# Diegotistical/OptionsLab

Hardware: AMD Instinct MI355X
Metric: MC path-steps/sec (1M paths × 252 steps Euro call); price vs BS |err|/σ (higher is better)
Workload: dtype f32 normals / f64 prices

## Files before the change

include/olmc.h:

```cpp
#ifndef OLMC_H
#define OLMC_H

#include <stdint.h>

#ifdef __cplusplus
extern "C" {
#endif

#define OLMC_ABI_VERSION 6

enum {
    OLMC_OK = 0,
    OLMC_ERR_ARG = 1,
    OLMC_ERR_HIP = 2,
    OLMC_ERR_STATE = 3,
    OLMC_ERR_RCCL = 4
};

enum { OLMC_STREAM_GBM = 0, OLMC_STREAM_HESTON = 1, OLMC_STREAM_JUMP = 2, OLMC_STREAM_KOU = 3 };
enum { OLMC_AVG_ARITHMETIC = 0, OLMC_AVG_GEOMETRIC = 1, OLMC_AVG_ARITHMETIC_FAST = 2 };
#define OLMC_MAX_BATCH 16

typedef struct olmc_stats {
    double  sum;
// ... 184 lines not shown
                       const uint32_t* sv, const uint32_t* shift, int32_t bits, int path_major, double* out_host);

int olmc_multi_gpu_european(double S, double K, double T, double r, double sigma, double q, int is_call,
                            int64_t n_paths, int32_t n_steps, uint64_t seed, int antithetic,
                            int n_gpus, olmc_stats* out);
int olmc_multi_gpu_greeks_fd(double S, double K, double T, double r, double sigma, double q, int is_call,
                             int64_t n_paths, int32_t n_steps, uint64_t seed, int second_order,
                             int n_gpus, double* out9, olmc_stats* evals );
int olmc_multi_gpu_european_cv(double S, double K, double T, double r, double sigma, double q, int is_call,
                               int64_t n_paths, int32_t n_steps, uint64_t seed, int antithetic,
                               int n_gpus, olmc_cv_moments* out);
int olmc_multi_gpu_european_qmc(double S, double K, double T, double r, double sigma, double q, int is_call,
                                int64_t n_paths, int32_t dims, const uint32_t* sv, const uint32_t* shift, int32_t bits,
                                int n_gpus, olmc_stats* out);
int olmc_multi_gpu_european_qmc_greeks_fd(double S, double K, double T, double r, double sigma, double q, int is_call,
                                          int64_t n_paths, int32_t dims, const uint32_t* sv, const uint32_t* shift, int32_t bits,
                                          int second_order, int n_gpus, double* out9, olmc_stats* evals );
int olmc_multi_gpu_european_qmc_cv(double S, double K, double T, double r, double sigma, double q, int is_call,
                                   int64_t n_paths, int32_t dims, const uint32_t* sv, const uint32_t* shift, int32_t bits,
                                   int n_gpus, olmc_cv_moments* out);
int olmc_multi_gpu_spans(double* out8);

int olmc_fetch_dev(const double* d_src, int32_t n, void* hip_stream, double* out_host);

int olmc_combine_stats(const olmc_stats* parts, int32_t n_parts, double r, double T, olmc_stats* out);

int olmc_philox_words(uint64_t seed, int64_t path_offset, int64_t n_paths,
                      int32_t block0, int32_t n_blocks, uint32_t stream_tag, uint32_t* out_host);
int olmc_normals(uint64_t seed, int64_t path_offset, int64_t n_paths, int32_t n_steps,
                 float* out_host);

int olmc_profile_enable(int on);
enum { OLMC_TUNE_GRID_CAP = 2, OLMC_TUNE_QMC_BLOCK = 4, OLMC_TUNE_SPLIT_TAIL = 7, OLMC_TUNE_POLL = 8, OLMC_TUNE_SPLIT_SAT = 9,
       OLMC_TUNE_MULTI_LAUNCH = 10, OLMC_TUNE_STAGED_COPY = 11 };
int olmc_tune(int knob, int value);
int olmc_profile_reset(void);
int olmc_kernel_time(int64_t* launches, double* total_ms);

#ifdef __cplusplus
}
#endif
#endif
```

optionslab_amd/_hip.py:

```python
from __future__ import annotations

import ctypes as C
import importlib.util
import os
import sys
import threading
from typing import List, Optional, Sequence, Tuple

import numpy as np

from .exceptions import AccelerationError

LIBRARY_PATH = os.environ.get("OLMC_LIBRARY") or os.path.join(os.path.dirname(os.path.abspath(__file__)), "libolmc.so")
MAX_BATCH = 16
AVG_ARITHMETIC, AVG_GEOMETRIC, AVG_ARITHMETIC_FAST = 0, 1, 2
_U64 = (1 << 64) - 1


class Stats(C.Structure):
    _fields_ = [("sum", C.c_double), ("sumsq", C.c_double), ("n", C.c_int64),
                ("price", C.c_double), ("std_error", C.c_double)]


class Option(C.Structure):
# ... 46 lines not shown
    "olmc_extrema_qmc": (_I, _SIX + [_I, _I, _D, _I, _I64, _I64, _I32, C.POINTER(C.c_uint32), C.POINTER(C.c_uint32), _I32, _I, C.POINTER(Stats)]),
    "olmc_asian_qmc_greeks_fd": (_I, _SIX + [_I, _I, _I, _I64, _I32, C.POINTER(C.c_uint32), C.POINTER(C.c_uint32), _I32, _I, _I, C.POINTER(_D), C.POINTER(Stats)]),
    "olmc_extrema_qmc_greeks_fd": (_I, _SIX + [_I, _I, _D, _I, _I64, _I32, C.POINTER(C.c_uint32), C.POINTER(C.c_uint32), _I32, _I, _I, C.POINTER(_D),
                                              C.POINTER(Stats)]),
    "olmc_asian_greeks_fd": (_I, _SIX + [_I, _I, _I64, _I32, _U64T, _I, _I, C.POINTER(_D), C.POINTER(Stats)]),
    "olmc_extrema_greeks_fd": (_I, _SIX + [_I, _I, _D, _I64, _I32, _U64T, _I, _I, C.POINTER(_D), C.POINTER(Stats)]),
    "olmc_barrier": (_I, _SIX + [_I, _D, _I, _I64, _I64, _I32, _U64T, _I, C.POINTER(Stats)]),
    "olmc_lookback": (_I, _SIX + [_I, _I, _I64, _I64, _I32, _U64T, _I, C.POINTER(Stats)]),
    "olmc_autocallable": (_I, [_D] * 9 + [_I32, _I64, _I64, _I32, _U64T, _I, C.POINTER(Stats)]),
    "olmc_cliquet": (_I, [_D] * 9 + [_I32, _I64, _I64, _I32, _U64T, _I, C.POINTER(Stats)]),
    "olmc_exercise_boundary": (_I, _SIX + [_I, _I64, _I32, _U64T, C.POINTER(_D)]),
    "olmc_heston_paths": (_I, [_D] * 9 + [_I64, _I32, _U64T, _I, C.POINTER(_D), C.POINTER(_D)]),
    "olmc_jump_paths": (_I, [_D] * 5 + [_I, _D, _D, _D, _D, _I64, _I32, _U64T, _I, C.POINTER(_D)]),
    "olmc_american_lsm": (_I, _SIX + [_I, _I64, _I32, _I32, _U64T, C.POINTER(Stats)]),
    "olmc_autocallable_qmc": (_I, [_D] * 9 + [_I32, _I, _I64, _I64, _I32, C.POINTER(C.c_uint32), C.POINTER(C.c_uint32), _I32, _I, C.POINTER(Stats)]),
    "olmc_cliquet_qmc": (_I, [_D] * 9 + [_I32, _I, _I64, _I64, _I32, C.POINTER(C.c_uint32), C.POINTER(C.c_uint32), _I32, _I, C.POINTER(Stats)]),
    "olmc_american_lsm_qmc": (_I, _SIX + [_I, _I, _I64, _I32, C.POINTER(C.c_uint32), C.POINTER(C.c_uint32), _I32, _I32, C.POINTER(Stats)]),
    "olmc_exercise_boundary_qmc": (_I, _SIX + [_I, _I, _I64, _I32, C.POINTER(C.c_uint32), C.POINTER(C.c_uint32), _I32, C.POINTER(_D)]),
    "olmc_gbm_qmc_paths": (_I, [_D] * 5 + [_I, _I64, _I32, C.POINTER(C.c_uint32), C.POINTER(C.c_uint32), _I32, _I, C.POINTER(_D)]),
    "olmc_jump_diffusion": (_I, _SIX + [_I, _I, _D, _D, _D, _D, _I64, _I64, _I32, _U64T, C.POINTER(Stats)]),
    "olmc_heston": (_I, [_D] * 5 + [_I] + [_D] * 5 + [_I64, _I64, _I32, _U64T, _I, C.POINTER(Stats)]),
    "olmc_multi_gpu_european": (_I, _SIX + [_I, _I64, _I32, _U64T, _I, _I, C.POINTER(Stats)]),
    "olmc_multi_gpu_greeks_fd": (_I, _SIX + [_I, _I64, _I32, _U64T, _I, _I, C.POINTER(_D), C.POINTER(Stats)]),
    "olmc_multi_gpu_european_cv": (_I, _SIX + [_I, _I64, _I32, _U64T, _I, _I, C.POINTER(CvMoments)]),
    "olmc_multi_gpu_european_qmc": (_I, _SIX + [_I, _I64, _I32, C.POINTER(C.c_uint32), C.POINTER(C.c_uint32), _I32, _I, C.POINTER(Stats)]),
    "olmc_multi_gpu_european_qmc_greeks_fd": (_I, _SIX + [_I, _I64, _I32, C.POINTER(C.c_uint32), C.POINTER(C.c_uint32), _I32, _I, _I, C.POINTER(_D), C.POINTER(Stats)]),
    "olmc_multi_gpu_european_qmc_cv": (_I, _SIX + [_I, _I64, _I32, C.POINTER(C.c_uint32), C.POINTER(C.c_uint32), _I32, _I, C.POINTER(CvMoments)]),
    "olmc_multi_gpu_spans": (_I, [C.POINTER(_D)]),
    "olmc_combine_stats": (_I, [C.POINTER(Stats), _I32, _D, _D, C.POINTER(Stats)]),
    "olmc_philox_words": (_I, [_U64T, _I64, _I64, _I32, _I32, C.c_uint32, C.POINTER(C.c_uint32)]),
    "olmc_normals": (_I, [_U64T, _I64, _I64, _I32, C.POINTER(C.c_float)]),
    "olmc_profile_enable": (_I, [_I]),
    "olmc_tune": (_I, [_I, _I]),
    "olmc_profile_reset": (_I, []),
    "olmc_kernel_time": (_I, [C.POINTER(_I64), C.POINTER(_D)]),
}

_lock = threading.Lock()
_lib: Optional[C.CDLL] = None
_initialised = False


def _share_hip_runtime_with_torch() -> None:
    if "torch" in sys.modules or os.environ.get("OLMC_SYSTEM_HIP") == "1":
        return
    try:
        spec = importlib.util.find_spec("torch")
    except (ImportError, ValueError):
        return
    if spec is None or not spec.submodule_search_locations:
        return
    cand = os.path.join(list(spec.submodule_search_locations)[0], "lib", "libamdhip64.so")
    if os.path.exists(cand):
        try:
            C.CDLL(cand, mode=C.RTLD_GLOBAL)
        except OSError:
            pass


def load_library() -> C.CDLL:
    global _lib
    with _lock:
        if _lib is None:
            _share_hip_runtime_with_torch()
            if not os.path.exists(LIBRARY_PATH):
                raise AccelerationError(
# ... 500 lines not shown
    _check(lib().olmc_multi_gpu_spans(out))
    return dict(zip(("launch_us", "collective_us", "fetch_us", "drain_us", "total_us", "wake_us_max", "rank_launch_us_max", "rank_launch_us_min"), out))


def combine_stats(parts: Sequence[Tuple[float, float, int]], r: float, T: float) -> Stats:
    k = len(parts)
    arr = (Stats * k)(*[Stats(s, ss, int(n), 0.0, 0.0) for (s, ss, n) in parts])
    out = Stats()
    _check(load_library().olmc_combine_stats(arr, k, r, T, C.byref(out)))
    return out


def philox_words(seed: int, path_offset: int, n_paths: int, block0: int, n_blocks: int, tag: int = 0) -> np.ndarray:
    out = np.empty((int(n_paths), int(n_blocks), 4), dtype=np.uint32)
    _check(lib().olmc_philox_words(seed64(seed), int(path_offset), int(n_paths), int(block0), int(n_blocks), int(tag),
                                   out.ctypes.data_as(C.POINTER(C.c_uint32))))
    return out


def normals(seed: int, path_offset: int, n_paths: int, n_steps: int) -> np.ndarray:
    out = np.empty((int(n_paths), int(n_steps)), dtype=np.float32)
    _check(lib().olmc_normals(seed64(seed), int(path_offset), int(n_paths), int(n_steps),
                              out.ctypes.data_as(C.POINTER(C.c_float))))
    return out


TUNE_GRID_CAP = 2
TUNE_QMC_BLOCK = 4
TUNE_SPLIT_TAIL = 7
TUNE_POLL = 8
TUNE_SPLIT_SAT = 9
TUNE_MULTI_LAUNCH = 10
TUNE_STAGED_COPY = 11


def tune(knob: int, value: int) -> None:
    _check(load_library().olmc_tune(int(knob), int(value)))


def profile_enable(on: bool) -> None:
    _check(lib().olmc_profile_enable(int(on)))


def profile_reset() -> None:
    _check(lib().olmc_profile_reset())


def kernel_time() -> Tuple[int, float]:
    n, ms = C.c_int64(0), C.c_double(0.0)
    _check(lib().olmc_kernel_time(C.byref(n), C.byref(ms)))
    return n.value, ms.value
```

optionslab_amd/csrc/olmc.hip:

```cpp
#include "olmc.h"
#include "olmc_kernels.h"
#include "olmc_job_board.h"

#include <dlfcn.h>
#include <sched.h>
#include <time.h>
#include <hip/hip_ext.h>
#include <rccl/rccl.h>

#include <algorithm>
#include <atomic>
#include <chrono>
#include <climits>
#include <condition_variable>
#include <cmath>
#include <cstdio>
#include <cstdlib>
#include <cstring>
#include <functional>
#include <mutex>
#include <string>
#include <system_error>
#include <thread>
#include <vector>
#include <linux/futex.h>
#include <sys/prctl.h>
#include <sys/syscall.h>
#include <unistd.h>

namespace {

using namespace olmc;

thread_local std::string t_error = "";
thread_local int t_device = -1;

int fail(int code, const std::string& msg) {
    t_error = msg;
    return code;
}

#define HIP_TRY(expr)                                                                          \
    do {                                                                                       \
        hipError_t e_ = (expr);                                                                \
        if (e_ != hipSuccess)                                                                  \
            return fail(OLMC_ERR_HIP, std::string(#expr) + ": " + hipGetErrorString(e_));      \
    } while (0)

constexpr int kMaxDevices = 16;
constexpr int kMaxNV = 2 * OLMC_MAX_BATCH;
constexpr int32_t kMaxGrid = 1 << 18;
constexpr int32_t kMaxGroups = kMaxGrid / kGroupBlocks + 1;
static_assert(kMaxGroups * kMaxNV == kGroupRowsCapacity, "device-side guard must match the group_rows allocation");

struct EventPair {
    hipEvent_t start, stop;
};

struct DeviceCtx {
    int device = -1;
    int cus = 0;
    hipStream_t stream = nullptr;
    struct WsSlot {
        double* block_rows = nullptr;
        size_t cap = 0;
        double* group_rows = nullptr;
        uint32_t* counters = nullptr;
        hipEvent_t done = nullptr;
        bool used = false;
        bool claimed = false;
        hipStream_t owner = nullptr;
        bool shared = false;
    };
    static constexpr int kSlots = 8;
    WsSlot slots[kSlots + 1];
    int next_slot = 0, cur_slot = 0;
    uint64_t* h_flag = nullptr;
    uint64_t* d_flag = nullptr;
    uint64_t seq = 0;
    uint64_t armed = 0;
    double* h_result = nullptr;
    double* d_result = nullptr;
    void* d_bulk = nullptr;
    size_t bulk_bytes = 0;
    void* h_stage[2] = {nullptr, nullptr};
    hipEvent_t stage_landed[2] = {nullptr, nullptr};
    void* d_multi = nullptr;
    void* h_multi = nullptr;
    void* d_h_multi = nullptr;
    int64_t multi_cap = 0;
    size_t multi_bpo = 0;
    size_t multi_off_done = 0, multi_off_opts = 0, multi_off_rows = 0, multi_hoff_out = 0;
    uint32_t* d_sobol = nullptr;
    size_t sobol_words = 0;
    std::vector<uint32_t> sobol_host;
    void* d_bridge = nullptr;
    int32_t bridge_n = 0;
    std::vector<unsigned char> bridge_host;
    bool busy = false;
    std::vector<EventPair> ev_free, ev_pending;
    int64_t prof_launches = 0;
    double prof_ms = 0.0;
};

constexpr int kMaxContexts = 8;

struct DevicePool {
    std::mutex mu;
    std::condition_variable idle;
    std::vector<DeviceCtx*> all;
    int device = -1;
};

std::mutex g_mu;
std::atomic<DevicePool*> g_pool[kMaxDevices] = {};
std::atomic<int> g_default_device{-1};
bool g_profile = false;

int ctx_allocate(DeviceCtx* c) {
    HIP_TRY(hipStreamCreateWithFlags(&c->stream, hipStreamNonBlocking));
    for (auto& sl : c->slots) {
        HIP_TRY(hipMalloc(&sl.group_rows, sizeof(double) * kMaxNV * kMaxGroups));
        HIP_TRY(hipMalloc(&sl.counters, sizeof(uint32_t) * (kMaxGroups + 1) * kCounterStride));
        HIP_TRY(hipMemset(sl.counters, 0, sizeof(uint32_t) * (kMaxGroups + 1) * kCounterStride));
        HIP_TRY(hipEventCreateWithFlags(&sl.done, hipEventDisableTiming));
    }
    HIP_TRY(hipHostMalloc(&c->h_result, sizeof(double) * (kMaxNV + 1 + 15), hipHostMallocMapped));
    HIP_TRY(hipHostGetDevicePointer(reinterpret_cast<void**>(&c->d_result), c->h_result, 0));
    c->h_flag = reinterpret_cast<uint64_t*>(c->h_result + kMaxNV + 8);
    c->d_flag = reinterpret_cast<uint64_t*>(c->d_result + kMaxNV + 8);
    *c->h_flag = 0;
    return OLMC_OK;
}

void ctx_release(DeviceCtx* c) {
    if (c->stream) (void)hipStreamSynchronize(c->stream);
    for (auto& ep : c->ev_pending) { (void)hipEventDestroy(ep.start); (void)hipEventDestroy(ep.stop); }
    for (auto& ep : c->ev_free) { (void)hipEventDestroy(ep.start); (void)hipEventDestroy(ep.stop); }
    if (c->d_bulk) (void)hipFree(c->d_bulk);
    for (int i = 0; i < 2; ++i) {
        if (c->h_stage[i]) (void)hipHostFree(c->h_stage[i]);
        if (c->stage_landed[i]) (void)hipEventDestroy(c->stage_landed[i]);
    }
    if (c->d_multi) (void)hipFree(c->d_multi);
    if (c->h_multi) (void)hipHostFree(c->h_multi);
    if (c->d_sobol) (void)hipFree(c->d_sobol);
    if (c->d_bridge) (void)hipFree(c->d_bridge);
    for (auto& sl : c->slots) {
        if (sl.block_rows) (void)hipFree(sl.block_rows);
        if (sl.group_rows) (void)hipFree(sl.group_rows);
        if (sl.counters) (void)hipFree(sl.counters);
        if (sl.done) (void)hipEventDestroy(sl.done);
    }
    if (c->h_result) (void)hipHostFree(c->h_result);
    if (c->stream) (void)hipStreamDestroy(c->stream);
    delete c;
}

int ctx_create(int device, DeviceCtx** out) {
    int count = 0;
    hipError_t e = hipGetDeviceCount(&count);
    if (e != hipSuccess || count <= 0)
        return fail(OLMC_ERR_HIP, std::string("no HIP device available: ") + hipGetErrorString(e));
    if (device < 0 || device >= count || device >= kMaxDevices)
        return fail(OLMC_ERR_ARG, "device index out of range");
    HIP_TRY(hipSetDevice(device));
    hipDeviceProp_t prop;
    HIP_TRY(hipGetDeviceProperties(&prop, device));
    DeviceCtx* c = new DeviceCtx();
    c->device = device;
    c->cus = prop.multiProcessorCount;
    const int rc = ctx_allocate(c);
    if (rc) {
        ctx_release(c);
        return rc;
    }
    *out = c;
    return OLMC_OK;
}

struct CtxLease {
    DeviceCtx* c = nullptr;
    DevicePool* pool = nullptr;
    CtxLease() = default;
    CtxLease(const CtxLease&) = delete;
    CtxLease& operator=(const CtxLease&) = delete;
    ~CtxLease() { release(); }
// ... 120 lines not shown
        if (err == hipSuccess) err = hipEventRecord(c->stage_landed[slot], c->stream);
        if (err == hipSuccess && i >= 1) {
            const auto t = clock::now();
            err = hipEventSynchronize(c->stage_landed[slot ^ 1]);
            if (i == 1) us_first = us_since(t); else us_events += us_since(t);
            if (err == hipSuccess) landed.store(i, std::memory_order_release);
        }
    }
    {
        const auto t = clock::now();
        if (err == hipSuccess) err = hipEventSynchronize(c->stage_landed[(n_chunks - 1) & 1]);
        us_events += us_since(t);
    }
    if (err == hipSuccess) landed.store(n_chunks, std::memory_order_release);
    else give_up.store(true);
    const auto t_join = clock::now();
    for (std::thread& t : threads) t.join();
    if (trace)
        std::fprintf(stderr, "[olmc copy_to_host] %.1f MB, %lld chunks, %d threads: spawn %.0f us, first chunk landed (kernel + DMA) %.0f us, later event waits %.0f us, "
                             "waits for the copy threads %.0f us, last chunk out + join %.0f us, total %.0f us\n", bytes / 1e6, static_cast<long long>(n_chunks), n_threads,
                     us_spawn, us_first, us_events, us_workers, us_since(t_join), us_since(t_begin));
    if (err != hipSuccess) {
        (void)hipStreamSynchronize(c->stream);
        (void)hipGetLastError();
        return fail(OLMC_ERR_HIP, std::string("copy_to_host: ") + hipGetErrorString(err));
    }
    return OLMC_OK;
}

int g_multi_launch = 0;
int g_grid_cap = 0;
int g_qmc_block = 0;
int g_poll = 0;
int g_split_tail = 0;
int g_split_sat = 0;
#ifdef OLMC_WITH_PROBES
int g_fault_shard = 0;
int g_force_nv = 0;
int g_multi_rehearsal = 0;
#endif

constexpr int32_t kShortPathSteps = 128, kShortPathGrid = 4096;

int32_t grid_for(int64_t n_paths, int32_t n_steps = INT32_MAX) {
    int64_t cap = g_grid_cap > 0 ? std::min<int64_t>(g_grid_cap, kMaxGrid) : kMaxGrid;
    if (g_grid_cap == 0 && n_steps <= kShortPathSteps) cap = kShortPathGrid;
    return static_cast<int32_t>(std::min<int64_t>((n_paths + kBlock - 1) / kBlock, cap));
}

template <typename Kernel>
int resident_workgroups(Kernel kernel) {
    static std::mutex mu;
    static std::vector<std::pair<const void*, int>> cache;
    const void* key = reinterpret_cast<const void*>(kernel);
    std::lock_guard<std::mutex> lock(mu);
    for (const auto& e : cache)
        if (e.first == key) return e.second;
    int nb = 0;
    if (hipOccupancyMaxActiveBlocksPerMultiprocessor(&nb, kernel, kBlock, 0) != hipSuccess || nb < 1) {
        (void)hipGetLastError();
        nb = 1;
    }
    cache.emplace_back(key, nb);
    return nb;
}

// ... 40 lines not shown
                HIP_TRY(hipDeviceSynchronize());
                taken.shared = true;
                taken.used = false;
            }
        }
    }
    DeviceCtx::WsSlot& sl = c->slots[idx];
    c->cur_slot = idx;
    const bool guarded = !own && sl.shared;
    const size_t need = static_cast<size_t>(grid) * nv;
    if (need > sl.cap) {
        if (!guarded) HIP_TRY(hipStreamSynchronize(stream));
        else if (sl.used) HIP_TRY(hipEventSynchronize(sl.done));
        if (sl.block_rows) HIP_TRY(hipFree(sl.block_rows));
        sl.block_rows = nullptr;
        sl.cap = 0;
        const size_t cap = std::max<size_t>(need, size_t(1) << 16);
        HIP_TRY(hipMalloc(&sl.block_rows, sizeof(double) * cap));
        sl.cap = cap;
    }
    if (guarded && sl.used) HIP_TRY(hipStreamWaitEvent(stream, sl.done, 0));
    ws->block_rows = sl.block_rows;
    ws->group_rows = sl.group_rows;
    ws->counters = sl.counters;
    ws->out = d_out;
    ws->tail = tail;
    ws->row_capacity = sl.cap;
#ifdef OLMC_WITH_PROBES
    if (g_force_nv > 0) ws->row_capacity = static_cast<uint64_t>(grid) * g_force_nv;
#endif
    ws->done_flag = nullptr;
    ws->done_value = 0;
    c->armed = 0;
    if (own && d_out == c->d_result && g_poll >= 0) {
        c->armed = ++c->seq;
        ws->done_flag = c->d_flag;
        ws->done_value = c->armed;
    }
    return OLMC_OK;
}

void ws_recover(DeviceCtx* c) {
    c->armed = 0;
    (void)hipDeviceSynchronize();
    (void)hipGetLastError();
    for (auto& sl : c->slots) (void)hipMemset(sl.counters, 0, sizeof(uint32_t) * (kMaxGroups + 1) * kCounterStride);
}

void multi_recover(DeviceCtx* c) {
    c->armed = 0;
    (void)hipDeviceSynchronize();
    (void)hipGetLastError();
    if (c->d_multi) (void)hipMemset(c->d_multi, 0, c->multi_off_opts);
}

int after_launch(DeviceCtx* c, hipStream_t stream) {
    hipError_t e = hipGetLastError();
    if (e != hipSuccess) { ws_recover(c); return fail(OLMC_ERR_HIP, std::string("kernel launch: ") + hipGetErrorString(e)); }
    if (c->cur_slot == DeviceCtx::kSlots || !c->slots[c->cur_slot].shared) return OLMC_OK;
    DeviceCtx::WsSlot& sl = c->slots[c->cur_slot];
    HIP_TRY(hipEventRecord(sl.done, stream));
    sl.used = true;
    return OLMC_OK;
}

int prof_begin(DeviceCtx* c, hipStream_t s, EventPair* ep) {
    if (c->ev_free.empty()) {
        HIP_TRY(hipEventCreate(&ep->start));
        HIP_TRY(hipEventCreate(&ep->stop));
    } else {
        *ep = c->ev_free.back();
        c->ev_free.pop_back();
    }
    HIP_TRY(hipEventRecord(ep->start, s));
    return OLMC_OK;
}
// ... 64 lines not shown
template <typename F>
void with_set_anti(int nsets, bool anti, F&& f) {
    with_bool(nsets == 8, [&](auto eight) { with_bool(anti, [&](auto a) { f(std::integral_constant<int, eight ? 8 : 16>{}, a); }); });
}

int prof_pair(DeviceCtx* c, EventPair* ep, const EventPair** timed) {
    *timed = nullptr;
    if (!g_profile) return OLMC_OK;
    int rc = prof_acquire(c, ep);
    if (rc) return rc;
    c->ev_pending.push_back(*ep);
    *timed = ep;
    return OLMC_OK;
}

template <int NSETS, int MODE>
void launch_european(bool anti, int32_t grid, hipStream_t s, const PathRange& pr, const ContractSet<NSETS>& cs,
                     const ReduceWs& ws, double* terminal, const EventPair* timed = nullptr) {
    const bool strided = static_cast<int64_t>(grid) * kBlock < pr.count;
    with_bool(strided, [&](auto strided_c) {
        with_bool(anti, [&](auto a) {
            launch_timed(european_path_kernel<NSETS, a, MODE, strided_c>, dim3(grid), dim3(kBlock), s, timed, pr, cs, ws, terminal);
        });
    });
}

int sync_or_recover(DeviceCtx* c, hipStream_t s);

template <typename Launch>
int launch_reduce(DeviceCtx* c, hipStream_t s, double* d_out, double tail, int nv, int32_t grid, Launch&& launch, bool profiled = true) {
    ReduceWs ws;
    int rc = make_ws(c, s, grid, nv, d_out, tail, &ws);
    if (rc) return rc;
    EventPair ep{};
    const EventPair* timed = nullptr;
    if (profiled) {
        rc = prof_pair(c, &ep, &timed);
        if (rc) return rc;
    }
    launch(grid, s, timed, ws);
    rc = after_launch(c, s);
    if (rc || d_out != c->d_result) return rc;
    return sync_or_recover(c, s);
}

void finish_one(const double* h, int64_t n, double r_disc, double T, bool bad, olmc_stats* out) {
    if (bad) nan_stats(n, out);
    else finish_stats(h[0], h[1], n, r_disc, T, out);
}

void finish_set(const double* h, const int* pos, int64_t n, const olmc_option* opts, int64_t k, bool extra_bad, bool lean, olmc_stats* st) {
    for (int64_t i = 0; i < k; ++i) {
        const int64_t slot = pos ? pos[i] : i;
        const olmc_option& o = opts[i];
        if (extra_bad || poisoned(o.S, o.K, o.T, o.r, o.sigma, o.q)) nan_stats(n, &st[i]);
        else if (lean) finish_stats(h[slot], std::nan(""), n, o.r, o.T, &st[i]);
        else finish_stats(h[2 * slot], h[2 * slot + 1], n, o.r, o.T, &st[i]);
    }
}

struct GbmStep {
    double dt, drift, vol;
};
GbmStep gbm_step(double T, int32_t n_steps, double r, double q, double sigma) {
    const double dt = T / n_steps;
    return {dt, (r - q - 0.5 * sigma * sigma) * dt, sigma * std::sqrt(dt)};
// ... 15 lines not shown
            ContractSet<width> cs;
            group_contracts<width>(opts, k, n_steps, &cs, pos);
            if (!lean) launch_european<width, kReduce>(anti, g, st, pr, cs, ws, nullptr, timed);
            else with_bool(anti, [&](auto a) { launch_timed(european_path_kernel<width, a, kSumOnly, false>, dim3(g), dim3(kBlock), st, timed, pr, cs, ws, nullptr); });
        };
        if (nsets == 1) {
            ContractSet<1> cs;
            cs.c[0] = make_contract(opts[0], n_steps);
            cs.base_mask = 1u; cs.upper_continues_slot0 = 0;
            if (pos) pos[0] = 0;
            launch_european<1, kReduce>(anti, g, st, pr, cs, ws, nullptr, timed);
        } else if (nsets == 8) {
            fused(std::integral_constant<int, 8>{});
        } else {
            fused(std::integral_constant<int, 16>{});
        }
    }, profiled);
}

constexpr int64_t kSpinUs = 200, kYieldUs = 2000, kSleepUs = 20;

struct TimerSlack {
    long old = -1;
    void tighten() {
        if (old >= 0) return;
        old = prctl(PR_GET_TIMERSLACK, 0, 0, 0, 0);
        if (old >= 0 && prctl(PR_SET_TIMERSLACK, 1000UL, 0, 0, 0) != 0) old = -1;
    }
    ~TimerSlack() {
        if (old >= 0) (void)prctl(PR_SET_TIMERSLACK, static_cast<unsigned long>(old), 0, 0, 0);
    }
};

int wait_armed(DeviceCtx* c, hipStream_t s) {
    if (c->armed != 0) {
        const uint64_t want = c->armed;
        c->armed = 0;
        using clock = std::chrono::steady_clock;
        const auto t0 = clock::now();
        bool queried = false;
        int phase = 0;
        TimerSlack slack;
        for (uint32_t spins = 0;; ++spins) {
            if (__atomic_load_n(c->h_flag, __ATOMIC_ACQUIRE) == want) {
                if (queried) (void)hipGetLastError();
                return OLMC_OK;
            }
            if (phase == 0) {
                __builtin_ia32_pause();
                if ((spins & 0x3F) == 0x3F && clock::now() - t0 >= std::chrono::microseconds(kSpinUs)) phase = 1;
                continue;
            }
            if (phase == 1) {
                sched_yield();
                if ((spins & 0xF) == 0xF && clock::now() - t0 >= std::chrono::microseconds(kYieldUs)) phase = 2;
                continue;
            }
            if ((spins & 0x3F) == 0) {
                const hipError_t q = hipStreamQuery(s);
                queried = true;
                if (q == hipSuccess) break;
                if (q != hipErrorNotReady) {
                    ws_recover(c);
                    return fail(OLMC_ERR_HIP, std::string("hipStreamQuery: ") + hipGetErrorString(q));
                }
            }
            slack.tighten();
            const timespec nap{0, kSleepUs * 1000};
            nanosleep(&nap, nullptr);
        }
        (void)hipGetLastError();
    }
    hipError_t e = hipStreamSynchronize(s);
    if (e != hipSuccess) { ws_recover(c); return fail(OLMC_ERR_HIP, std::string("hipStreamSynchronize: ") + hipGetErrorString(e)); }
    return OLMC_OK;
}

int sync_or_recover(DeviceCtx* c, hipStream_t s) {
    if (s != c->stream) c->armed = 0;
    return wait_armed(c, s);
}

int run_batch(const olmc_option* opts, int32_t k, int64_t path_offset, int64_t n_local, int32_t n_steps,
              uint64_t seed, int antithetic, olmc_stats* out, bool prices_only = false) {
    if (!opts || !out) return fail(OLMC_ERR_ARG, "null pointer");
    if (k < 1 || k > OLMC_MAX_BATCH) return fail(OLMC_ERR_ARG, "batch size must be in [1, OLMC_MAX_BATCH]");
    int rc = check_paths(path_offset, n_local, n_steps);
    if (rc) return rc;
    CtxLease lease;
    rc = ctx_lease(&lease);
    if (rc) return rc;
    DeviceCtx* const c = lease.c;
    int pos[OLMC_MAX_BATCH];
    bool lean = prices_only;
    rc = run_batch_device(c, c->stream, opts, k, path_offset, n_local, n_steps, seed, antithetic, c->d_result, -1.0, pos, true, &lean);
    if (rc) return rc;
    finish_set(c->h_result, pos, n_local * (antithetic ? 2 : 1), opts, k, false, lean, out);
    return OLMC_OK;
}

}

namespace { void multi_gpu_release(); }

extern "C" int olmc_abi_version(void) { return OLMC_ABI_VERSION; }

extern "C" const char* olmc_last_error(void) { return t_error.c_str(); }

extern "C" int olmc_init(int device) {
    std::lock_guard<std::mutex> lock(g_mu);
    static const bool env_read = [] {
        const char* p = std::getenv("OLMC_POLL");
        if (p && p[0] == '0') g_poll = -1;
        const char* t = std::getenv("OLMC_SPLIT_TAIL");
        if (t && t[0] == '0') g_split_tail = -1;
        const char* m = std::getenv("OLMC_MULTI_LAUNCH");
        if (m && m[0] == 's') g_multi_launch = -1;
        const char* sc = std::getenv("OLMC_STAGED_COPY");
        if (sc && sc[0] == '0') g_staged_copy = -1;
        return true;
    }();
    (void)env_read;
    if (device < 0 || device >= kMaxDevices) return fail(OLMC_ERR_ARG, "device index out of range");
    if (!g_pool[device].load(std::memory_order_acquire)) {
        DeviceCtx* c = nullptr;
        int rc = ctx_create(device, &c);
        if (rc) return rc;
        DevicePool* pool = new DevicePool();
        pool->device = device;
        pool->all.push_back(c);
        g_pool[device].store(pool, std::memory_order_release);
    } else {
        HIP_TRY(hipSetDevice(device));
    }
    t_device = device;
    if (g_default_device.load() < 0) g_default_device.store(device, std::memory_order_release);
    return OLMC_OK;
}

extern "C" int olmc_shutdown(void) {
    std::lock_guard<std::mutex> lock(g_mu);
    multi_gpu_release();
    for (int d = 0; d < kMaxDevices; ++d) {
        DevicePool* pool = g_pool[d].load();
        if (!pool) continue;
        const bool usable = hipSetDevice(d) == hipSuccess;
// ... 1843 lines not shown
    rc = bulk_reserve(c, bytes);
    if (rc) return rc;
    const int64_t total = n_paths * n_blocks;
    const int grid = static_cast<int>(std::min<int64_t>((total + 255) / 256, 4096));
    hipLaunchKernelGGL(philox_words_kernel, dim3(grid), dim3(256), 0, c->stream, static_cast<uint64_t>(path_offset), n_paths,
                       block0, n_blocks, stream_tag, static_cast<uint32_t>(seed), static_cast<uint32_t>(seed >> 32),
                       static_cast<uint32_t*>(c->d_bulk));
    HIP_TRY(hipGetLastError());
    HIP_TRY(hipMemcpyAsync(out_host, c->d_bulk, bytes, hipMemcpyDeviceToHost, c->stream));
    HIP_TRY(hipStreamSynchronize(c->stream));
    return OLMC_OK;
}

extern "C" int olmc_normals(uint64_t seed, int64_t path_offset, int64_t n_paths, int32_t n_steps, float* out_host) {
    if (!out_host || n_paths < 1 || n_steps < 1 || path_offset < 0) return fail(OLMC_ERR_ARG, "bad arguments");
    CtxLease lease;
    int rc = ctx_lease(&lease);
    if (rc) return rc;
    DeviceCtx* const c = lease.c;
    const size_t bytes = sizeof(float) * static_cast<size_t>(n_paths) * n_steps;
    rc = bulk_reserve(c, bytes);
    if (rc) return rc;
    const int64_t total = n_paths * ((n_steps + 3) / 4);
    const int grid = static_cast<int>(std::min<int64_t>((total + 255) / 256, 4096));
    hipLaunchKernelGGL(normals_kernel, dim3(grid), dim3(256), 0, c->stream, static_cast<uint64_t>(path_offset), n_paths,
                       n_steps, static_cast<uint32_t>(seed), static_cast<uint32_t>(seed >> 32),
                       static_cast<float*>(c->d_bulk));
    HIP_TRY(hipGetLastError());
    HIP_TRY(hipMemcpyAsync(out_host, c->d_bulk, bytes, hipMemcpyDeviceToHost, c->stream));
    HIP_TRY(hipStreamSynchronize(c->stream));
    return OLMC_OK;
}

extern "C" int olmc_tune(int knob, int value) {
    if (knob == OLMC_TUNE_GRID_CAP && value >= 0) { g_grid_cap = value; return OLMC_OK; }
    if (knob == OLMC_TUNE_QMC_BLOCK && value >= -1 && value <= 2) { g_qmc_block = value; return OLMC_OK; }
    if (knob == OLMC_TUNE_POLL && value >= -1 && value <= 0) { g_poll = value; return OLMC_OK; }
    if (knob == OLMC_TUNE_SPLIT_TAIL && value >= -1 && value <= 0) { g_split_tail = value; return OLMC_OK; }
    if (knob == OLMC_TUNE_SPLIT_SAT && value >= 0 && value <= 16) { g_split_sat = value; return OLMC_OK; }
    if (knob == OLMC_TUNE_MULTI_LAUNCH && value >= -1 && value <= 0) { g_multi_launch = value; return OLMC_OK; }
    if (knob == OLMC_TUNE_STAGED_COPY && value >= -1 && value <= 0) { g_staged_copy = value; return OLMC_OK; }
    return fail(OLMC_ERR_ARG, "unknown tuning knob or value");
}

namespace {
template <typename Fn>
int with_all_contexts(Fn fn) {
    int dev = t_device >= 0 ? t_device : g_default_device.load(std::memory_order_acquire);
    if (dev < 0) {
        int rc = olmc_init(0);
        if (rc) return rc;
        dev = t_device;
    }
    DevicePool* pool = g_pool[dev].load(std::memory_order_acquire);
    if (!pool) return fail(OLMC_ERR_STATE, "device not initialised (call olmc_init)");
    HIP_TRY(hipSetDevice(dev));
    std::vector<DeviceCtx*> mine;
    {
        std::unique_lock<std::mutex> lock(pool->mu);
        pool->idle.wait(lock, [&] { return std::none_of(pool->all.begin(), pool->all.end(), [](const DeviceCtx* c) { return c->busy; }); });
        mine = pool->all;
        for (DeviceCtx* c : mine) c->busy = true;
    }
    int rc = OLMC_OK;
    for (DeviceCtx* c : mine) {
        const int r = fn(c);
        if (r && !rc) rc = r;
    }
    {
        std::lock_guard<std::mutex> lock(pool->mu);
// ... 50 lines not shown
```

optionslab_amd/csrc/olmc_host_math.h:

```cpp
#ifndef OLMC_HOST_MATH_H
#define OLMC_HOST_MATH_H

#include "olmc.h"

#include <algorithm>
#include <cmath>
#include <cstdint>
#include <cstring>

namespace olmc {

struct Contract {
    double a;
    double vol;
    double strike;
    double sign;
    double scale;
    double neg_sign_strike;
    double sign_scale;
};

template <int NSETS>
struct ContractSet {
    Contract c[NSETS];
// ... 306 lines not shown
            if (n_groups == real_slots) return "more distinct path recursions than the fused Asian Greeks kernel carries";
            as->drift[g] = drift;
            as->vol[g] = vol;
            ++n_groups;
        }
        as->group[i] = g;
    }
    for (int g = n_groups; g < kAsianGroups; ++g) { as->drift[g] = as->drift[0]; as->vol[g] = as->vol[0]; }
    for (int g = 0; g < kAsianGroups; ++g) {
        as->drift[g] = as->drift[g] * unit;
        as->vol[g] = as->vol[g] * kZScale * unit;
    }
    as->strike = K;
    as->sign = is_call ? 1.0 : -1.0;
    as->inv_steps = 1.0 / n_steps;
    return nullptr;
}

inline void shard_range(int64_t n_paths, int rank, int n_ranks, int64_t* lo, int64_t* count) {
    const int64_t a = n_paths * rank / n_ranks, b = n_paths * (rank + 1) / n_ranks;
    *lo = a;
    *count = b - a;
}

constexpr int64_t kQmcShardAlign = 512, kQmcShardMinPoints = 4096;
inline void qmc_shard_range(int64_t n_points, int rank, int n_ranks, int64_t* lo, int64_t* count) {
    if (n_points / n_ranks < kQmcShardMinPoints) return shard_range(n_points, rank, n_ranks, lo, count);
    const int64_t a = n_points * rank / n_ranks / kQmcShardAlign * kQmcShardAlign;
    const int64_t b = rank + 1 == n_ranks ? n_points : n_points * (rank + 1) / n_ranks / kQmcShardAlign * kQmcShardAlign;
    *lo = a;
    *count = b - a;
}

}

#endif
```

optionslab_amd/csrc/olmc_kernels.h:

```cpp
#pragma once
#include <type_traits>
#include <hip/hip_runtime.h>
#include <stdint.h>

#include "olmc_host_math.h"

namespace olmc {

constexpr int kBlock = 256;
constexpr int kWave = 64;
constexpr int kWavesPerBlock = kBlock / kWave;

constexpr uint32_t kPhiloxM0 = 0xD2511F53u;
constexpr uint32_t kPhiloxM1 = 0xCD9E8D57u;
constexpr uint32_t kPhiloxW0 = 0x9E3779B9u;
constexpr uint32_t kPhiloxW1 = 0xBB67AE85u;

struct Words4 {
    uint32_t x0, x1, x2, x3;
};

__device__ __forceinline__ uint32_t xor3(uint32_t a, uint32_t b, uint32_t c) {
    return __builtin_amdgcn_bitop3_b32(a, b, c, 0x96);
}
// ... 119 lines not shown
            float s = 0.0f;
            for (; b < full; ++b) s = raw_block_sum_of_words(s, philox4x32_10_pinned(g_lo, g_hi, static_cast<uint32_t>(b), tag, rk));
            q += static_cast<double>(s);
        }
        const int32_t rem = n_steps & 3;
        if (rem) {
            const Words4 wd = philox4x32_10_pinned(g_lo, g_hi, static_cast<uint32_t>(full), tag, rk);
            float s = 0.0f;
            if (rem > 1) s = pair_sum_raw(0.0f, wd.x0, wd.x1);
            if (rem & 1) {
                float z_cos, z_sin;
                box_muller_raw(rem == 1 ? wd.x0 : wd.x2, rem == 1 ? wd.x1 : wd.x3, z_cos, z_sin);
                s = __builtin_fmaf(z_cos, kInvSqrt2F, s);
            }
            q += static_cast<double>(s);
        }
        acc += q;
    }
    return acc;
}

__device__ __forceinline__ double path_normal_sum(uint32_t g_lo, uint32_t g_hi, int32_t n_steps, uint32_t k0, uint32_t k1,
                                                  uint32_t tag = 0u) {
    return path_normal_quarters(g_lo, g_hi, n_steps, 0, 4, k0, k1, tag) * kPairZScale;
}

__device__ __forceinline__ double wave_sum(double v) {
#pragma unroll
    for (int off = kWave / 2; off > 0; off >>= 1) v += __shfl_down(v, off, kWave);
    return v;
}

constexpr int kGroupBlocks = 256;
constexpr int kGroupRowsCapacity = ((1 << 18) / kGroupBlocks + 1) * 32;
constexpr int kCounterStride = 64;

struct ReduceWs {
    double* block_rows;
    double* group_rows;
    uint32_t* counters;
    double* out;
    double tail;
    uint64_t row_capacity;
    uint64_t* done_flag;
    uint64_t done_value;
};

__device__ __forceinline__ void signal_done(const ReduceWs& ws) {
    if (ws.done_flag == nullptr) return;
    __builtin_amdgcn_fence(__ATOMIC_RELEASE, "");
    if (threadIdx.x == 0) __hip_atomic_store(ws.done_flag, ws.done_value, __ATOMIC_RELAXED, __HIP_MEMORY_SCOPE_SYSTEM);
}

#ifndef OLMC_AGENT_ACQUIRE
#define OLMC_AGENT_ACQUIRE 1
#endif
#if !OLMC_AGENT_ACQUIRE && defined(__HIP_DEVICE_COMPILE__) && !defined(__gfx942__) && !defined(__gfx950__)
#error "OLMC_AGENT_ACQUIRE=0 relies on gfx942 / gfx950 cache behaviour (sc1 rows are L2-served): build this target with the acquire"
#endif
__device__ __forceinline__ void acquire_rows() {
#if OLMC_AGENT_ACQUIRE
    __builtin_amdgcn_fence(__ATOMIC_ACQUIRE, "agent");
#else
    __builtin_amdgcn_fence(__ATOMIC_ACQUIRE, "wavefront");
#endif
}

__device__ __forceinline__ void store_sc1(double* p, double v) {
    __hip_atomic_store(p, v, __ATOMIC_RELAXED, __HIP_MEMORY_SCOPE_AGENT);
}
__device__ __forceinline__ double load_sc1(const double* p) {
    return __hip_atomic_load(p, __ATOMIC_RELAXED, __HIP_MEMORY_SCOPE_AGENT);
}

template <int NV>
__device__ __forceinline__ double wave_rows_sum(const double* src, int32_t rows) {
    constexpr int NVP = NV <= 2 ? 2 : NV <= 8 ? 8 : NV <= 16 ? 16 : 32;
    constexpr int SUBS = kWave / NVP;
    const int lane = threadIdx.x & (kWave - 1);
    const int c = lane % NVP, sub = lane / NVP;
    double v = 0.0;
    if (c < NV) {
        constexpr int kBatch = 8;
        for (int32_t row = sub; row < rows; row += SUBS * kBatch) {
// ... 1 lines not shown
#pragma unroll
            for (int j = 0; j < kBatch; ++j) {
                const int32_t rj = row + j * SUBS;
                t[j] = rj < rows ? load_sc1(src + static_cast<size_t>(rj) * NV + c) : 0.0;
            }
#pragma unroll
            for (int j = 0; j < kBatch; ++j) v += t[j];
        }
    }
#pragma unroll
    for (int off = kWave / 2; off >= NVP; off >>= 1) v += __shfl_down(v, off, kWave);
    return v;
}

struct NoEpilogue {
    __device__ __forceinline__ void operator()(double) const {}
};

template <int NV, typename Epilogue = NoEpilogue>
__device__ __forceinline__ void grid_reduce(double v, const ReduceWs& ws, Epilogue done = Epilogue()) {
    const int lane = threadIdx.x;
    const int32_t n_blocks = static_cast<int32_t>(gridDim.x);
    const int32_t n_groups = (n_blocks + kGroupBlocks - 1) / kGroupBlocks;
    const int32_t group = static_cast<int32_t>(blockIdx.x) / kGroupBlocks;
    const int32_t group_size = min(kGroupBlocks, n_blocks - group * kGroupBlocks);

    if (static_cast<uint64_t>(n_blocks) * NV > ws.row_capacity || n_groups * NV > kGroupRowsCapacity) {
        if (blockIdx.x == 0) {
            if (lane < NV) ws.out[lane] = __builtin_nan("");
            signal_done(ws);
        }
        return;
    }
    if (lane < NV) store_sc1(ws.block_rows + static_cast<size_t>(blockIdx.x) * NV + lane, v);
    asm volatile("s_waitcnt vmcnt(0)" ::: "memory");
    uint32_t ticket = 0;
    if (lane == 0) ticket = __hip_atomic_fetch_add(ws.counters + static_cast<size_t>(group) * kCounterStride, 1u, __ATOMIC_RELAXED, __HIP_MEMORY_SCOPE_AGENT);
    ticket = __builtin_amdgcn_readfirstlane(ticket);
    if (ticket != static_cast<uint32_t>(group_size - 1)) return;

    acquire_rows();
    const double g = wave_rows_sum<NV>(ws.block_rows + static_cast<size_t>(group) * kGroupBlocks * NV, group_size);
    if (n_groups == 1) {
        if (lane < NV) ws.out[lane] = g;
        if (lane == 0) {
            if (ws.tail >= 0.0) ws.out[NV] = ws.tail;
            __hip_atomic_store(ws.counters, 0u, __ATOMIC_RELAXED, __HIP_MEMORY_SCOPE_AGENT);
        }
        done(g);
        signal_done(ws);
        return;
    }
    if (lane < NV) store_sc1(ws.group_rows + static_cast<size_t>(group) * NV + lane, g);
    asm volatile("s_waitcnt vmcnt(0)" ::: "memory");
    if (lane == 0) {
        __hip_atomic_store(ws.counters + static_cast<size_t>(group) * kCounterStride, 0u, __ATOMIC_RELAXED, __HIP_MEMORY_SCOPE_AGENT);
        ticket = __hip_atomic_fetch_add(ws.counters + static_cast<size_t>(n_groups) * kCounterStride, 1u, __ATOMIC_RELAXED, __HIP_MEMORY_SCOPE_AGENT);
    }
    ticket = __builtin_amdgcn_readfirstlane(ticket);
    if (ticket != static_cast<uint32_t>(n_groups - 1)) return;

    acquire_rows();
    const double total = wave_rows_sum<NV>(ws.group_rows, n_groups);
    if (lane < NV) ws.out[lane] = total;
    if (lane == 0) {
        if (ws.tail >= 0.0) ws.out[NV] = ws.tail;
// ... 20 lines not shown
            }
#pragma unroll
            for (int j = 0; j < kBatch; ++j) v += t[j];
        }
    }
    part[threadIdx.x] = v;
    __syncthreads();
    double total = 0.0;
    if (threadIdx.x < NV) {
#pragma unroll
        for (int k = 0; k < SUBS; ++k) total += part[k * NVP + threadIdx.x];
    }
    __syncthreads();
    return total;
}

template <int NV, typename Epilogue = NoEpilogue>
__device__ __forceinline__ void grid_reduce_workgroup(double v, const ReduceWs& ws, Epilogue done = Epilogue()) {
    __shared__ double part[kBlock];
    __shared__ uint32_t last;
    const int t = threadIdx.x;
    const bool wave0 = t < kWave;
    const int32_t n_blocks = static_cast<int32_t>(gridDim.x);
    const int32_t n_groups = (n_blocks + kGroupBlocks - 1) / kGroupBlocks;
    const int32_t group = static_cast<int32_t>(blockIdx.x) / kGroupBlocks;
    const int32_t group_size = min(kGroupBlocks, n_blocks - group * kGroupBlocks);

    if (static_cast<uint64_t>(n_blocks) * NV > ws.row_capacity || n_groups * NV > kGroupRowsCapacity) {
        if (blockIdx.x == 0 && wave0) {
            if (t < NV) ws.out[t] = __builtin_nan("");
            signal_done(ws);
        }
        return;
    }
    if (wave0) {
        if (t < NV) store_sc1(ws.block_rows + static_cast<size_t>(blockIdx.x) * NV + t, v);
        asm volatile("s_waitcnt vmcnt(0)" ::: "memory");
        if (t == 0) last = __hip_atomic_fetch_add(ws.counters + static_cast<size_t>(group) * kCounterStride, 1u, __ATOMIC_RELAXED, __HIP_MEMORY_SCOPE_AGENT) ==
                           static_cast<uint32_t>(group_size - 1);
    }
    __syncthreads();
    if (!last) return;

    acquire_rows();
    const double g = workgroup_rows_sum<NV>(ws.block_rows + static_cast<size_t>(group) * kGroupBlocks * NV, group_size, part);
    if (n_groups == 1) {
        if (wave0) {
            if (t < NV) ws.out[t] = g;
            if (t == 0) {
                if (ws.tail >= 0.0) ws.out[NV] = ws.tail;
                __hip_atomic_store(ws.counters, 0u, __ATOMIC_RELAXED, __HIP_MEMORY_SCOPE_AGENT);
            }
            done(g);
            signal_done(ws);
        }
        return;
    }
    if (wave0) {
        if (t < NV) store_sc1(ws.group_rows + static_cast<size_t>(group) * NV + t, g);
        asm volatile("s_waitcnt vmcnt(0)" ::: "memory");
        if (t == 0) {
            __hip_atomic_store(ws.counters + static_cast<size_t>(group) * kCounterStride, 0u, __ATOMIC_RELAXED, __HIP_MEMORY_SCOPE_AGENT);
            last = __hip_atomic_fetch_add(ws.counters + static_cast<size_t>(n_groups) * kCounterStride, 1u, __ATOMIC_RELAXED, __HIP_MEMORY_SCOPE_AGENT) ==
                   static_cast<uint32_t>(n_groups - 1);
        }
    }
// ... 2540 lines not shown
```

Measured before the change: 2447 billion.

## Hand per-block partial sums to the host via tagged mapped memory

Instead of the device doing a grid-wide ticketed reduction (atomic counters, last-block group sums, done flag), each block writes its partial sum as a value/tag word pair directly into coherent mapped host memory. The host poller then collects the words as they arrive and replays the device's summation order on the CPU, so it can return as soon as all rows have landed. This removes the atomic ticket and final-reduction tail from the kernel. In exchange it adds per-block system-scope stores, host-side polling and summation work, and a fallback path when rows are missing.

```diff
diff --git a/include/olmc.h b/include/olmc.h
--- a/include/olmc.h
+++ b/include/olmc.h
@@ -240,8 +240,9 @@
 
 int olmc_profile_enable(int on);
 enum { OLMC_TUNE_GRID_CAP = 2, OLMC_TUNE_QMC_BLOCK = 4, OLMC_TUNE_SPLIT_TAIL = 7, OLMC_TUNE_POLL = 8, OLMC_TUNE_SPLIT_SAT = 9,
-       OLMC_TUNE_MULTI_LAUNCH = 10, OLMC_TUNE_STAGED_COPY = 11 };
+       OLMC_TUNE_MULTI_LAUNCH = 10, OLMC_TUNE_STAGED_COPY = 11, OLMC_TUNE_HOST_ROWS = 12 };
 int olmc_tune(int knob, int value);
+int64_t olmc_host_sum_launches(void);
 int olmc_profile_reset(void);
 int olmc_kernel_time(int64_t* launches, double* total_ms);
 
diff --git a/optionslab_amd/_hip.py b/optionslab_amd/_hip.py
--- a/optionslab_amd/_hip.py
+++ b/optionslab_amd/_hip.py
@@ -102,6 +102,7 @@
     "olmc_normals": (_I, [_U64T, _I64, _I64, _I32, C.POINTER(C.c_float)]),
     "olmc_profile_enable": (_I, [_I]),
     "olmc_tune": (_I, [_I, _I]),
+    "olmc_host_sum_launches": (_I64, []),
     "olmc_profile_reset": (_I, []),
     "olmc_kernel_time": (_I, [C.POINTER(_I64), C.POINTER(_D)]),
 }
@@ -668,10 +669,15 @@
 TUNE_SPLIT_SAT = 9
 TUNE_MULTI_LAUNCH = 10
 TUNE_STAGED_COPY = 11
+TUNE_HOST_ROWS = 12
 
 
 def tune(knob: int, value: int) -> None:
     _check(load_library().olmc_tune(int(knob), int(value)))
+
+
+def host_sum_launches() -> int:
+    return int(load_library().olmc_host_sum_launches())
 
 
 def profile_enable(on: bool) -> None:
diff --git a/optionslab_amd/csrc/olmc.hip b/optionslab_amd/csrc/olmc.hip
--- a/optionslab_amd/csrc/olmc.hip
+++ b/optionslab_amd/csrc/olmc.hip
@@ -51,6 +51,8 @@
 constexpr int kMaxNV = 2 * OLMC_MAX_BATCH;
 constexpr int32_t kMaxGrid = 1 << 18;
 constexpr int32_t kMaxGroups = kMaxGrid / kGroupBlocks + 1;
+constexpr uint64_t kHostRowWords = uint64_t(1) << 17;
+static_assert(kMaxNV <= kRowsMaxNV, "the host replay's widest row");
 static_assert(kMaxGroups * kMaxNV == kGroupRowsCapacity, "device-side guard must match the group_rows allocation");
 
 struct EventPair {
@@ -80,6 +82,12 @@
     uint64_t seq = 0;
     uint64_t armed = 0;
     double* h_result = nullptr;
+    HostRowWord* h_rows = nullptr;
+    HostRowWord* d_rows = nullptr;
+    int32_t rows_grid = 0;
+    int rows_nv = 0;
+    std::vector<double> rows_vals, rows_groups;
+    std::vector<int32_t> rows_next, rows_open;
     double* d_result = nullptr;
     void* d_bulk = nullptr;
     size_t bulk_bytes = 0;
@@ -130,6 +138,9 @@
     c->h_flag = reinterpret_cast<uint64_t*>(c->h_result + kMaxNV + 8);
     c->d_flag = reinterpret_cast<uint64_t*>(c->d_result + kMaxNV + 8);
     *c->h_flag = 0;
+    HIP_TRY(hipHostMalloc(reinterpret_cast<void**>(&c->h_rows), sizeof(HostRowWord) * kHostRowWords, hipHostMallocMapped | hipHostMallocCoherent));
+    HIP_TRY(hipHostGetDevicePointer(reinterpret_cast<void**>(&c->d_rows), c->h_rows, 0));
+    std::memset(c->h_rows, 0, sizeof(HostRowWord) * kHostRowWords);
     return OLMC_OK;
 }
 
@@ -153,6 +164,7 @@
         if (sl.done) (void)hipEventDestroy(sl.done);
     }
     if (c->h_result) (void)hipHostFree(c->h_result);
+    if (c->h_rows) (void)hipHostFree(c->h_rows);
     if (c->stream) (void)hipStreamDestroy(c->stream);
     delete c;
 }
@@ -339,6 +351,8 @@
 int g_grid_cap = 0;
 int g_qmc_block = 0;
 int g_poll = 0;
+int g_host_rows = 0;
+std::atomic<int64_t> g_host_sum_launches{0};
 int g_split_tail = 0;
 int g_split_sat = 0;
 #ifdef OLMC_WITH_PROBES
@@ -445,6 +459,7 @@
     ws->done_flag = nullptr;
     ws->done_value = 0;
     c->armed = 0;
+    c->rows_grid = 0;
     if (own && d_out == c->d_result && g_poll >= 0) {
         c->armed = ++c->seq;
         ws->done_flag = c->d_flag;
@@ -453,8 +468,24 @@
     return OLMC_OK;
 }
 
+void arm_host_rows(DeviceCtx* c, int32_t grid, int nv, double tail, ReduceWs* ws) {
+    if (c->armed == 0 || g_host_rows < 0 || tail >= 0.0 || nv < 1 || nv > kRowsMaxNV) return;
+    const uint64_t cap = g_host_rows > 0 ? std::min<uint64_t>(g_host_rows, kHostRowWords) : kHostRowWords;
+    if (static_cast<uint64_t>(grid) * nv > cap) return;
+    ws->block_rows = reinterpret_cast<double*>(c->d_rows);
+    ws->counters = nullptr;
+    ws->group_rows = nullptr;
+#ifdef OLMC_WITH_PROBES
+    if (g_force_nv <= 0)
+#endif
+    ws->row_capacity = cap;
+    c->rows_grid = grid;
+    c->rows_nv = nv;
+}
+
 void ws_recover(DeviceCtx* c) {
     c->armed = 0;
+    c->rows_grid = 0;
     (void)hipDeviceSynchronize();
     (void)hipGetLastError();
     for (auto& sl : c->slots) (void)hipMemset(sl.counters, 0, sizeof(uint32_t) * (kMaxGroups + 1) * kCounterStride);
@@ -585,6 +616,7 @@
     ReduceWs ws;
     int rc = make_ws(c, s, grid, nv, d_out, tail, &ws);
     if (rc) return rc;
+    arm_host_rows(c, grid, nv, tail, &ws);
     EventPair ep{};
     const EventPair* timed = nullptr;
     if (profiled) {
@@ -666,7 +698,45 @@
     }
 };
 
+struct RowsConsumer {
+    DeviceCtx* c;
+    uint64_t seq;
+    int32_t grid, n_groups;
+    int nv;
+    RowsConsumer(DeviceCtx* ctx, uint64_t want) : c(ctx), seq(want), grid(ctx->rows_grid), n_groups(rows_groups(ctx->rows_grid)), nv(ctx->rows_nv) {
+        c->rows_grid = 0;
+        if (grid == 0) return;
+        const size_t words = static_cast<size_t>(grid) * nv;
+        if (c->rows_vals.size() < words) c->rows_vals.resize(words);
+        if (c->rows_groups.size() < static_cast<size_t>(n_groups) * nv) c->rows_groups.resize(static_cast<size_t>(n_groups) * nv);
+        c->rows_next.assign(n_groups, 0);
+        c->rows_open.resize(n_groups);
+        for (int32_t g = 0; g < n_groups; ++g) c->rows_open[g] = g;
+    }
+    bool active() const { return grid != 0; }
+    bool poll() {
+        std::vector<int32_t>& open = c->rows_open;
+        for (size_t k = 0; k < open.size();) {
+            const int32_t g = open[k], size = std::min<int32_t>(kRowsGroup, grid - g * kRowsGroup), words = size * nv;
+            const size_t base = static_cast<size_t>(g) * kRowsGroup * nv;
+            int32_t i = c->rows_next[g];
+            while (i < words && take_host_word(c->h_rows + base + i, seq, &c->rows_vals[base + i])) ++i;
+            c->rows_next[g] = i;
+            if (i < words) { ++k; continue; }
+            rows_sum_host(&c->rows_vals[base], size, nv, &c->rows_groups[static_cast<size_t>(g) * nv]);
+            open[k] = open.back();
+            open.pop_back();
+        }
+        if (!open.empty()) return false;
+        g_host_sum_launches.fetch_add(1, std::memory_order_relaxed);
+        if (n_groups == 1) for (int m = 0; m < nv; ++m) c->h_result[m] = c->rows_groups[m];
+        else rows_sum_host(c->rows_groups.data(), n_groups, nv, c->h_result);
+        return true;
+    }
+};
+
 int wait_armed(DeviceCtx* c, hipStream_t s) {
+    RowsConsumer rows(c, c->armed);
     if (c->armed != 0) {
         const uint64_t want = c->armed;
         c->armed = 0;
@@ -676,7 +746,7 @@
         int phase = 0;
         TimerSlack slack;
         for (uint32_t spins = 0;; ++spins) {
-            if (__atomic_load_n(c->h_flag, __ATOMIC_ACQUIRE) == want) {
+            if ((rows.active() && rows.poll()) || __atomic_load_n(c->h_flag, __ATOMIC_ACQUIRE) == want) {
                 if (queried) (void)hipGetLastError();
                 return OLMC_OK;
             }
@@ -704,6 +774,13 @@
             nanosleep(&nap, nullptr);
         }
         (void)hipGetLastError();
+        hipError_t e = hipStreamSynchronize(s);
+        if (e != hipSuccess) { ws_recover(c); return fail(OLMC_ERR_HIP, std::string("hipStreamSynchronize: ") + hipGetErrorString(e)); }
+        if (rows.active() && !rows.poll() && __atomic_load_n(c->h_flag, __ATOMIC_ACQUIRE) != want) {
+            ws_recover(c);
+            return fail(OLMC_ERR_STATE, "the launch retired without handing all of its rows to the host");
+        }
+        return OLMC_OK;
     }
     hipError_t e = hipStreamSynchronize(s);
     if (e != hipSuccess) { ws_recover(c); return fail(OLMC_ERR_HIP, std::string("hipStreamSynchronize: ") + hipGetErrorString(e)); }
@@ -746,6 +823,8 @@
     static const bool env_read = [] {
         const char* p = std::getenv("OLMC_POLL");
         if (p && p[0] == '0') g_poll = -1;
+        const char* hr = std::getenv("OLMC_HOST_ROWS");
+        if (hr && hr[0] == '0') g_host_rows = -1;
         const char* t = std::getenv("OLMC_SPLIT_TAIL");
         if (t && t[0] == '0') g_split_tail = -1;
         const char* m = std::getenv("OLMC_MULTI_LAUNCH");
@@ -2655,10 +2734,13 @@
     return OLMC_OK;
 }
 
+extern "C" int64_t olmc_host_sum_launches(void) { return g_host_sum_launches.load(std::memory_order_relaxed); }
+
 extern "C" int olmc_tune(int knob, int value) {
     if (knob == OLMC_TUNE_GRID_CAP && value >= 0) { g_grid_cap = value; return OLMC_OK; }
     if (knob == OLMC_TUNE_QMC_BLOCK && value >= -1 && value <= 2) { g_qmc_block = value; return OLMC_OK; }
     if (knob == OLMC_TUNE_POLL && value >= -1 && value <= 0) { g_poll = value; return OLMC_OK; }
+    if (knob == OLMC_TUNE_HOST_ROWS && value >= -1) { g_host_rows = value; return OLMC_OK; }
     if (knob == OLMC_TUNE_SPLIT_TAIL && value >= -1 && value <= 0) { g_split_tail = value; return OLMC_OK; }
     if (knob == OLMC_TUNE_SPLIT_SAT && value >= 0 && value <= 16) { g_split_sat = value; return OLMC_OK; }
     if (knob == OLMC_TUNE_MULTI_LAUNCH && value >= -1 && value <= 0) { g_multi_launch = value; return OLMC_OK; }
diff --git a/optionslab_amd/csrc/olmc_host_math.h b/optionslab_amd/csrc/olmc_host_math.h
--- a/optionslab_amd/csrc/olmc_host_math.h
+++ b/optionslab_amd/csrc/olmc_host_math.h
@@ -362,6 +362,67 @@
     *count = b - a;
 }
 
+constexpr int kRowsWave = 64, kRowsBlock = 256, kRowsGroup = 256;
+constexpr int kRowsMaxNV = 32;
+
+struct alignas(16) HostRowWord {
+    uint64_t value;
+    uint64_t tag;
+};
+
+inline bool take_host_word(const HostRowWord* w, uint64_t seq, double* out) {
+    const uint64_t value = __atomic_load_n(&w->value, __ATOMIC_RELAXED), tag = __atomic_load_n(&w->tag, __ATOMIC_RELAXED);
+    if ((value ^ tag) != seq) return false;
+    std::memcpy(out, &value, sizeof value);
+    return true;
+}
+
+inline double rows_lane_sum(const double* src, int32_t rows, int nv, int c, int32_t first, int32_t stride, int batch) {
+    double v = 0.0;
+    for (int32_t row = first; row < rows; row += stride * batch)
+        for (int j = 0; j < batch; ++j) {
+            const int32_t rj = row + j * stride;
+            v += rj < rows ? src[static_cast<size_t>(rj) * nv + c] : 0.0;
+        }
+    return v;
+}
+
+inline void wave_rows_sum_host(const double* src, int32_t rows, int nv, double* out) {
+    const int nvp = nv <= 2 ? 2 : nv <= 8 ? 8 : nv <= 16 ? 16 : 32, subs = kRowsWave / nvp;
+    double v[kRowsWave];
+    for (int lane = 0; lane < kRowsWave; ++lane) {
+        const int c = lane % nvp, sub = lane / nvp;
+        v[lane] = c < nv ? rows_lane_sum(src, rows, nv, c, sub, subs, 8) : 0.0;
+    }
+    for (int off = kRowsWave / 2; off >= nvp; off >>= 1)
+        for (int lane = 0; lane < kRowsWave; ++lane) v[lane] = v[lane] + (lane + off < kRowsWave ? v[lane + off] : v[lane]);
+    for (int c = 0; c < nv; ++c) out[c] = v[c];
+}
+
+inline void workgroup_rows_sum_host(const double* src, int32_t rows, int nv, double* out) {
+    const int nvp = nv <= 8 ? 8 : nv <= 16 ? 16 : 32, subs = kRowsBlock / nvp, batch = nvp >= 16 ? 16 : 8;
+    for (int c = 0; c < nv; ++c) {
+        double total = 0.0;
+        for (int k = 0; k < subs; ++k) total += rows_lane_sum(src, rows, nv, c, k, subs, batch);
+        out[c] = total;
+    }
+}
+
+inline void rows_sum_host(const double* src, int32_t rows, int nv, double* out) {
+    if (nv <= 2) wave_rows_sum_host(src, rows, nv, out);
+    else workgroup_rows_sum_host(src, rows, nv, out);
+}
+
+inline int32_t rows_groups(int32_t n_blocks) { return (n_blocks + kRowsGroup - 1) / kRowsGroup; }
+
+inline void grid_rows_total_host(const double* rows, int32_t n_blocks, int nv, double* group_rows, double* out) {
+    const int32_t n_groups = rows_groups(n_blocks);
+    for (int32_t g = 0; g < n_groups; ++g)
+        rows_sum_host(rows + static_cast<size_t>(g) * kRowsGroup * nv, std::min<int32_t>(kRowsGroup, n_blocks - g * kRowsGroup), nv, group_rows + static_cast<size_t>(g) * nv);
+    if (n_groups == 1) for (int c = 0; c < nv; ++c) out[c] = group_rows[c];
+    else rows_sum_host(group_rows, n_groups, nv, out);
+}
+
 }
 
 #endif
diff --git a/optionslab_amd/csrc/olmc_kernels.h b/optionslab_amd/csrc/olmc_kernels.h
--- a/optionslab_amd/csrc/olmc_kernels.h
+++ b/optionslab_amd/csrc/olmc_kernels.h
@@ -175,6 +175,7 @@
 }
 
 constexpr int kGroupBlocks = 256;
+static_assert(kWave == kRowsWave && kBlock == kRowsBlock && kGroupBlocks == kRowsGroup, "olmc_host_math.h replays these sums with the device's shapes");
 constexpr int kGroupRowsCapacity = ((1 << 18) / kGroupBlocks + 1) * 32;
 constexpr int kCounterStride = 64;
 
@@ -187,12 +188,21 @@
     uint64_t row_capacity;
     uint64_t* done_flag;
     uint64_t done_value;
+    __device__ __forceinline__ bool host_sums() const { return counters == nullptr; }
+    __device__ __forceinline__ HostRowWord* host_rows() const { return reinterpret_cast<HostRowWord*>(block_rows); }
 };
 
 __device__ __forceinline__ void signal_done(const ReduceWs& ws) {
     if (ws.done_flag == nullptr) return;
     __builtin_amdgcn_fence(__ATOMIC_RELEASE, "");
     if (threadIdx.x == 0) __hip_atomic_store(ws.done_flag, ws.done_value, __ATOMIC_RELAXED, __HIP_MEMORY_SCOPE_SYSTEM);
+}
+
+__device__ __forceinline__ void store_host_word(HostRowWord* p, double v, uint64_t seq) {
+    typedef uint32_t u32x4 __attribute__((ext_vector_type(4)));
+    const uint64_t bits = static_cast<uint64_t>(__double_as_longlong(v)), tag = bits ^ seq;
+    const u32x4 w = {static_cast<uint32_t>(bits), static_cast<uint32_t>(bits >> 32), static_cast<uint32_t>(tag), static_cast<uint32_t>(tag >> 32)};
+    asm volatile("global_store_dwordx4 %0, %1, off sc0 sc1" ::"v"(p), "v"(w) : "memory");
 }
 
 #ifndef OLMC_AGENT_ACQUIRE
@@ -260,6 +270,12 @@
         }
         return;
     }
+    if constexpr (std::is_same<Epilogue, NoEpilogue>::value) {
+        if (ws.host_sums()) {
+            if (lane < NV) store_host_word(ws.host_rows() + static_cast<size_t>(blockIdx.x) * NV + lane, v, ws.done_value);
+            return;
+        }
+    }
     if (lane < NV) store_sc1(ws.block_rows + static_cast<size_t>(blockIdx.x) * NV + lane, v);
     asm volatile("s_waitcnt vmcnt(0)" ::: "memory");
     uint32_t ticket = 0;
@@ -346,6 +362,12 @@
             signal_done(ws);
         }
         return;
+    }
+    if constexpr (std::is_same<Epilogue, NoEpilogue>::value) {
+        if (ws.host_sums()) {
+            if (t < NV) store_host_word(ws.host_rows() + static_cast<size_t>(blockIdx.x) * NV + t, v, ws.done_value);
+            return;
+        }
     }
     if (wave0) {
         if (t < NV) store_sc1(ws.block_rows + static_cast<size_t>(blockIdx.x) * NV + t, v);
```

Result: faster. 2487 billion, median of 4 (+1.7%).
